# nagadomi/nunif

Hardware: NVIDIA H100
Metric: waifu2x_input_megapixels_per_sec (higher is better)
Workload: dtype f16

## Files before the change

### nunif_b200/csrc/gemm_wgmma.cuh

```cuda
#pragma once
#include "common.cuh"
#include "ptx.cuh"
#include <cuda.h>

namespace nb200 {

enum : int { ACT_NONE = 0, ACT_LRELU01 = 1, ACT_GELU = 2, ACT_RELU = 3 };
enum : int { OUT_NHWC = 0, OUT_PIXSHUF2 = 1, OUT_SPLIT = 2 };

struct GemmParams {
    int B, Ho, Wo, TH, TW, tiles_x, tiles_y;
    int N;
    int taps, cpt;
    int8_t tap_dx[16], tap_dy[16], tap_dyi[16];
    int n_tiles;
    const float* bias;
    int act;
    int out_mode, cout;
    int has_res, res_cy, res_cx;
    int res_before_act;
    int k2;
};

struct GemmMaps {
    CUtensorMap a, b;
    CUtensorMap o[4];
    union {
        CUtensorMap r[4];
        CUtensorMap a2;
    };
};

__device__ __forceinline__ void mbar_init(uint64_t* bar, uint32_t count) {
    asm volatile("mbarrier.init.shared::cta.b64 [%0], %1;" ::"r"(smem_u32(bar)), "r"(count));
}
__device__ __forceinline__ void mbar_expect_tx(uint64_t* bar, uint32_t bytes) {
    asm volatile("mbarrier.arrive.expect_tx.shared::cta.b64 _, [%0], %1;" ::"r"(smem_u32(bar)), "r"(bytes) : "memory");
}
__device__ __forceinline__ void mbar_arrive(uint64_t* bar) {
    asm volatile("mbarrier.arrive.shared::cta.b64 _, [%0];" ::"r"(smem_u32(bar)) : "memory");
}
static __device__ __noinline__ void mbar_timeout() {
    printf("nb200: mbarrier wait timed out (block %d,%d thread %d)\n", blockIdx.x, blockIdx.y, threadIdx.x);
    __trap();
}
__device__ __forceinline__ void mbar_wait(uint64_t* bar, uint32_t parity) {
    const uint32_t addr = smem_u32(bar);
    uint32_t done = 0;
#pragma unroll 1
    for (uint32_t it = 0; it < (1u << 18); ++it) {
        asm volatile(
            "{\n\t.reg .pred p;\n\t"
            "mbarrier.try_wait.parity.shared::cta.b64 p, [%1], %2, %3;\n\t"
            "selp.u32 %0, 1, 0, p;\n\t}"
            : "=r"(done) : "r"(addr), "r"(parity), "r"(20000u) : "memory");
        if (done) return;
    }
    mbar_timeout();
}
__device__ __forceinline__ void fence_barrier_init() {
    asm volatile("fence.mbarrier_init.release.cluster;" ::: "memory");
    asm volatile("fence.proxy.async.shared::cta;" ::: "memory");
}
__device__ __forceinline__ void tma_load_5d(const CUtensorMap* map, uint64_t* bar, void* dst, int c0, int c1, int c2, int c3, int c4) {
    asm volatile(
        "cp.async.bulk.tensor.5d.shared::cluster.global.tile.mbarrier::complete_tx::bytes [%0], [%1, {%3, %4, %5, %6, %7}], [%2];"
        ::"r"(smem_u32(dst)), "l"(map), "r"(smem_u32(bar)), "r"(c0), "r"(c1), "r"(c2), "r"(c3), "r"(c4) : "memory");
}
__device__ __forceinline__ void tma_load_2d(const CUtensorMap* map, uint64_t* bar, void* dst, int c0, int c1) {
    asm volatile(
        "cp.async.bulk.tensor.2d.shared::cluster.global.tile.mbarrier::complete_tx::bytes [%0], [%1, {%3, %4}], [%2];"
        ::"r"(smem_u32(dst)), "l"(map), "r"(smem_u32(bar)), "r"(c0), "r"(c1) : "memory");
}
__device__ __forceinline__ void tma_load_4d(const CUtensorMap* map, uint64_t* bar, void* dst, int c0, int c1, int c2, int c3) {
    asm volatile(
        "cp.async.bulk.tensor.4d.shared::cluster.global.tile.mbarrier::complete_tx::bytes [%0], [%1, {%3, %4, %5, %6}], [%2];"
        ::"r"(smem_u32(dst)), "l"(map), "r"(smem_u32(bar)), "r"(c0), "r"(c1), "r"(c2), "r"(c3) : "memory");
}
__device__ __forceinline__ void tma_store_4d(const CUtensorMap* map, const void* src, int c0, int c1, int c2, int c3) {
    asm volatile("cp.async.bulk.tensor.4d.global.shared::cta.tile.bulk_group [%0, {%2, %3, %4, %5}], [%1];"
                 ::"l"(map), "r"(smem_u32(src)), "r"(c0), "r"(c1), "r"(c2), "r"(c3) : "memory");
}
__device__ __forceinline__ void tma_store_2d(const CUtensorMap* map, const void* src, int c0, int c1) {
    asm volatile("cp.async.bulk.tensor.2d.global.shared::cta.tile.bulk_group [%0, {%2, %3}], [%1];"
                 ::"l"(map), "r"(smem_u32(src)), "r"(c0), "r"(c1) : "memory");
}
__device__ __forceinline__ void tma_store_commit() { asm volatile("cp.async.bulk.commit_group;" ::: "memory"); }
__device__ __forceinline__ void tma_store_wait_read() { asm volatile("cp.async.bulk.wait_group.read 0;" ::: "memory"); }
__device__ __forceinline__ void fence_async_smem() { asm volatile("fence.proxy.async.shared::cta;" ::: "memory"); }
__device__ __forceinline__ void consumer_bar_sync() { asm volatile("bar.sync 1, 256;" ::: "memory"); }
__device__ __forceinline__ void tma_prefetch_desc(const CUtensorMap* map) {
    asm volatile("prefetch.tensormap [%0];" ::"l"(map) : "memory");
}
__device__ __forceinline__ bool elect_one() {
    uint32_t pred;
    asm volatile(
        "{\n\t.reg .pred p;\n\t"
        "elect.sync _|p, 0xffffffff;\n\t"
        "selp.u32 %0, 1, 0, p;\n\t}"
        : "=r"(pred));
    return pred != 0;
}
__device__ __forceinline__ void wgmma_fence() { asm volatile("wgmma.fence.sync.aligned;" ::: "memory"); }
__device__ __forceinline__ void wgmma_commit() { asm volatile("wgmma.commit_group.sync.aligned;" ::: "memory"); }
template <int N>
__device__ __forceinline__ void wgmma_wait() { asm volatile("wgmma.wait_group.sync.aligned %0;" ::"n"(N) : "memory"); }
template <int K>
__device__ __forceinline__ void wgmma_fence_operands(float (&d)[K]) {
#pragma unroll
    for (int j = 0; j < K; ++j) asm volatile("" : "+f"(d[j])::"memory");
}
// ... 256 lines not shown
```

### nunif_b200/csrc/swin_attention_mma.cu

```cuda
#include "common.cuh"
#include "gemm_wgmma.cuh"
#include "swin_kernels.h"
#include "tmap.h"
#include <map>
#include <mutex>

namespace nb200 {

extern int g_tune[16];

namespace {
constexpr int WS = 6, WTOK = 36, WPAD = 48, HEADS = 6;
}

constexpr int NKT = 5;

template <int D>
struct AttnCtx {
    __half* sq;
    const int* sreg;
    const float4* bf;
    const __half* kbase[NKT];
    const __half* vbase[3];
    int hc, g, t4;
// ... 189 lines not shown
    }
    frag[i] = make_float4(v[0], v[1], v[2], v[3]);
}

int build_bias_frag(cudaStream_t st, const float* table, float* frag) {
    build_bias_frag_kernel<<<(HEADS * 3 * 6 * 32 + 255) / 256, 256, 0, st>>>(table, reinterpret_cast<float4*>(frag));
    NB_LAUNCHED();
    return 0;
}

template <int D>
static size_t attn_smem_bytes() {
    constexpr int C = D * HEADS, LD = C + 8;
    return (size_t)3 * WTOK * LD * 2 + (WTOK + WPAD) * 4 + 16;
}

static int set_attn_attrs(const void* func, size_t smem, int carveout) {
    static std::mutex mu;
    static std::map<std::pair<int, const void*>, int> done;
    int dev = 0;
    NB_CUDA(cudaGetDevice(&dev));
    std::lock_guard<std::mutex> lk(mu);
    int& have = done[{dev, func}];
    if (have != carveout) {
        NB_CUDA(cudaFuncSetAttribute(func, cudaFuncAttributeMaxDynamicSharedMemorySize, (int)smem));
        NB_CUDA(cudaFuncSetAttribute(func, cudaFuncAttributePreferredSharedMemoryCarveout, carveout));
        have = carveout;
    }
    return 0;
}

int window_attention(cudaStream_t st, const __half* qkv, const float* bias_frag_f, __half* out, int B, int H, int W, int C,
                     int shift, size_t plane) {
    const float4* bias_table = reinterpret_cast<const float4*>(bias_frag_f);
    NB_CHECK(H % WS == 0 && W % WS == 0, "feature map must be a multiple of the 6x6 window");
    NB_CHECK(C == 96 || C == 192, "window attention supports C=96 (d=16) and C=192 (d=32)");
    if (WS >= H) shift = 0;
    dim3 grid((H / WS) * (W / WS), B);
    ProfScope ps(st, PC_ATTN, (double)B * H * W * C * 4 * 2, (double)B * H * W * C * 3 * 2, (double)B * H * W * C * 2);
    if (C == 96) {
        const int want = g_tune[6] > 0 ? g_tune[6] : 72;
        if (set_attn_attrs((const void*)window_attention_mma_kernel<16>, attn_smem_bytes<16>(), want)) return 1;
        window_attention_mma_kernel<16><<<grid, 192, attn_smem_bytes<16>(), st>>>(qkv, bias_table, out, H, W, shift, plane);
    } else {
        const int want = g_tune[6] > 0 ? g_tune[6] : 86;
        if (set_attn_attrs((const void*)window_attention_mma_kernel<32>, attn_smem_bytes<32>(), want)) return 1;
        window_attention_mma_kernel<32><<<grid, 192, attn_smem_bytes<32>(), st>>>(qkv, bias_table, out, H, W, shift, plane);
    }
    NB_LAUNCHED();
    return 0;
}


constexpr int FA_ROWS = 128, FA_WIN = 3, FA_THREADS = GEMM_CONSUMER_THREADS + 32, FA_SLOT = 96 * 64, FA_STAGES = 4;
constexpr int FA_LD = 32 + 8;
constexpr int FA_CHUNK_BYTES = FA_WIN * 3 * WTOK * FA_LD * 2;

template <int C>
struct FaCfg {
    static constexpr int X_BYTES = FA_ROWS * C * 2;
    static constexpr int SMEM = X_BYTES + FA_STAGES * FA_SLOT + FA_CHUNK_BYTES + FA_WIN * (WTOK + WPAD) * 4 + 2 * FA_STAGES * 8 + 1024;
};

template <int C>
__global__ void __launch_bounds__(FA_THREADS, 2) swin_attn_fused_kernel(const __grid_constant__ CUtensorMap wmap,
                                                                        const __half* __restrict__ x, const float* __restrict__ bqkv,
                                                                        const float4* __restrict__ bias_frag, __half* __restrict__ out,
                                                                        int H, int W, int shift, int nwin) {
    using Cfg = FaCfg<C>;
    constexpr int D = C / HEADS, KB = C / 32, NCH = C / 32, HPC = 32 / D;
    extern __shared__ uint8_t smem_dyn[];
    uint8_t* smem = reinterpret_cast<uint8_t*>((reinterpret_cast<uintptr_t>(smem_dyn) + 1023) & ~(uintptr_t)1023);
    uint8_t* sx = smem;
    uint8_t* ring = smem + Cfg::X_BYTES;
    __half* sqkv = reinterpret_cast<__half*>(ring + FA_STAGES * FA_SLOT);
    int* stok = reinterpret_cast<int*>(reinterpret_cast<uint8_t*>(sqkv) + FA_CHUNK_BYTES);
    int* sreg = stok + FA_WIN * WTOK;
    uint64_t* full = reinterpret_cast<uint64_t*>(sreg + FA_WIN * WPAD);
    uint64_t* empty = full + FA_STAGES;
    const int tid = threadIdx.x, warp = tid >> 5;
    const int nww = W / WS, nwy = H / WS;
    if (tid < FA_WIN * WPAD) {
        const int w = tid / WPAD, t = tid % WPAD, gw = blockIdx.x * FA_WIN + w;
        int reg = -1;
        if (t < WTOK) {
            int tok = -1;
            if (gw < nwin) {
                const int b = gw / (nww * nwy), r = gw % (nww * nwy), wy = r / nww, wx = r % nww;
                const int ry = wy * WS + t / WS, rx = wx * WS + t % WS;
                const int y = (ry + shift) % H, xx = (rx + shift) % W;
                tok = (b * H + y) * W + xx;
                int hr = 0, wr = 0;
                if (shift > 0) {
                    hr = ry < H - WS ? 0 : (ry < H - shift ? 1 : 2);
                    wr = rx < W - WS ? 0 : (rx < W - shift ? 1 : 2);
                }
                reg = hr * 3 + wr;
            }
            stok[w * WTOK + t] = tok;
        }
        sreg[w * WPAD + t] = reg;
    }
    if (tid == GEMM_CONSUMER_THREADS) {
        tma_prefetch_desc(&wmap);
        for (int s = 0; s < FA_STAGES; ++s) {
            mbar_init(&full[s], 1);
            mbar_init(&empty[s], 2);
        }
        fence_barrier_init();
    }
    __syncthreads();
    if (tid == 0) NB_PDL_TRIGGER();

    if (warp == GEMM_CONSUMER_THREADS / 32) {
        if (elect_one()) {
            for (int i = 0; i < NCH * KB; ++i) {
                const int s = i % FA_STAGES, c = i / KB;
                mbar_wait(&empty[s], ((i / FA_STAGES) & 1) ^ 1);
                mbar_expect_tx(&full[s], FA_SLOT);
#pragma unroll
                for (int m = 0; m < 3; ++m)
                    tma_load_2d(&wmap, &full[s], ring + s * FA_SLOT + m * 32 * 64, (i % KB) * 32, m * C + 32 * c);
            }
        }
        return;
    }

    for (int i = tid; i < FA_ROWS * (C / 8); i += GEMM_CONSUMER_THREADS) {
        const int r = i / (C / 8), u = i % (C / 8);
        uint8_t* dst = sx + (u >> 2) * (FA_ROWS * 64) + stage_off<32>(r, u & 3);
        const int tok = r < FA_WIN * WTOK ? stok[r] : -1;
        if (tok >= 0) cp_async16(dst, x + (size_t)tok * C + u * 8);
        else *reinterpret_cast<uint4*>(dst) = make_uint4(0u, 0u, 0u, 0u);
    }
    cp_async_commit();
    cp_async_wait<0>();
    fence_async_smem();
    consumer_bar_sync();

    const int wg = tid >> 7, t = tid & 127;
    const int row0 = wg * 64 + (t >> 5) * 16 + ((t & 31) >> 2);
    const int cq = 2 * (t & 3);
    const uint32_t a_base = smem_u32(sx) + wg * 64 * 64;
    const int lane = tid & 31, g = lane >> 2, t4 = lane & 3;
    const float scale = ((D == 16) ? 0.25f : 0.17677669529663687f) * 1.4426950408889634f;
#pragma unroll 1
    for (int c = 0; c < NCH; ++c) {
        float acc[48];
#pragma unroll
        for (int j = 0; j < 48; ++j) acc[j] = 0.f;
#pragma unroll 1
        for (int kb = 0; kb < KB; ++kb) {
            const int it = c * KB + kb, s = it % FA_STAGES;
            mbar_wait(&full[s], (it / FA_STAGES) & 1);
            const uint32_t a = a_base + kb * (FA_ROWS * 64), bb = smem_u32(ring + s * FA_SLOT);
            wgmma_fence();
            wgmma_f16<96>(acc, make_kmajor_desc<64>(a), make_kmajor_desc<64>(bb), 1u);
            wgmma_f16<96>(acc, make_kmajor_desc<64>(a + 32), make_kmajor_desc<64>(bb + 32), 1u);
            wgmma_commit();
            wgmma_wait<1>();
            if (kb > 0 && t == 0) mbar_arrive(&empty[(it - 1) % FA_STAGES]);
        }
        wgmma_wait<0>();
        if (t == 0) mbar_arrive(&empty[(c * KB + KB - 1) % FA_STAGES]);
        wgmma_fence_operands(acc);
        consumer_bar_sync();
#pragma unroll
        for (int j = 0; j < 12; ++j) {
            const int m = j >> 2, col = 8 * (j & 3) + cq;
            const float2 bq = __ldg(reinterpret_cast<const float2*>(bqkv + m * C + 32 * c + col));
#pragma unroll
            for (int i = 0; i < 2; ++i) {
                const int r = row0 + 8 * i;
                if (r < FA_WIN * WTOK) {
                    const int w = r / WTOK, tk = r - w * WTOK;
                    *reinterpret_cast<__half2*>(sqkv + ((w * 3 + m) * WTOK + tk) * FA_LD + col) =
                        __floats2half2_rn(acc[4 * j + 2 * i] + bq.x, acc[4 * j + 2 * i + 1] + bq.y);
                }
            }
        }
        consumer_bar_sync();

#pragma unroll 1
        for (int item = warp; item < 3 * FA_WIN * HPC; item += GEMM_CONSUMER_THREADS / 32) {
            const int mt = item / (FA_WIN * HPC), pr = item - mt * (FA_WIN * HPC), w = pr / HPC, hh = pr - w * HPC;
            const int gw = blockIdx.x * FA_WIN + w;
            if (gw >= nwin) continue;
            const int r = gw % (nww * nwy), wy = r / nww, wx = r % nww, head = c * HPC + hh;
            __half* sq = sqkv + w * 3 * WTOK * FA_LD;
            __half* sk = sq + WTOK * FA_LD;
            __half* sv = sk + WTOK * FA_LD;
            AttnCtx<D> cx;
            cx.sq = sq; cx.sreg = sreg + w * WPAD; cx.bf = bias_frag + (size_t)head * (3 * 6 * 32) + lane;
            cx.hc = hh * D; cx.g = g; cx.t4 = t4; cx.scale = scale;
            cx.boundary = shift > 0 && (wy == nwy - 1 || wx == nww - 1);
#pragma unroll
            for (int nt = 0; nt < NKT; ++nt) cx.kbase[nt] = sk + min(nt * 8 + g, WTOK - 1) * FA_LD + cx.hc + 2 * t4;
            cx.vbase[0] = sv + (lane & 15) * FA_LD + cx.hc;
            cx.vbase[1] = sv + (16 + (lane & 15)) * FA_LD + cx.hc;
            cx.vbase[2] = sv + min(32 + (lane & 7), WTOK - 1) * FA_LD + cx.hc;
            if (mt < 2) attn_mtile<D, FA_LD, false>(cx, mt);
            else attn_mtile<D, FA_LD, true>(cx, 2);
            __syncwarp();
            const int nrow = mt < 2 ? 16 : WTOK - 32;
            for (int e = lane; e < nrow * (D / 8); e += 32) {
                const int tk = 16 * mt + e / (D / 8), u = e % (D / 8);
                *reinterpret_cast<uint4*>(out + (size_t)stok[w * WTOK + tk] * C + head * D + u * 8) =
                    *reinterpret_cast<const uint4*>(sq + tk * FA_LD + cx.hc + u * 8);
            }
        }
    }
}

int swin_attn_fused(cudaStream_t st, const __half* x, const __half* wqkv, const float* bqkv, const float* bias_frag_f, __half* att,
                    int B, int H, int W, int C, int shift) {
    NB_CHECK(x && wqkv && bqkv && bias_frag_f && att, "null pointer");
    NB_CHECK(H % WS == 0 && W % WS == 0, "feature map must be a multiple of the 6x6 window");
    NB_CHECK(C == 96 || C == 192, "fused window attention supports C=96 (d=16) and C=192 (d=32)");
    if (WS >= H) shift = 0;
    const long long nwin = (long long)B * (H / WS) * (W / WS);
    NB_CHECK(nwin > 0 && nwin < (1LL << 31), "window count out of range");
    CUtensorMap wmap;
    const cuuint64_t dims[2] = {(cuuint64_t)C, (cuuint64_t)(3 * C)};
    const cuuint64_t strides[1] = {(cuuint64_t)C * 2};
    const cuuint32_t box[2] = {32, 32};
    if (encode(&wmap, wqkv, 2, dims, strides, box, 64)) return 1;
    const double T = (double)B * H * W;
    ProfScope ps(st, PC_FUSED_ATTN, T * 3.0 * C * C * 2 + T * C * 36 * 4, T * C * 2, T * C * 2);
    const unsigned grid = (unsigned)((nwin + FA_WIN - 1) / FA_WIN);
    if (rec_on()) {
        char line[96];
        snprintf(line, sizeof(line), "swin_attn,%d,%d,%d,%d,%d", B, H, W, C, shift);
        rec_append(line);
    }
    const float4* bf = reinterpret_cast<const float4*>(bias_frag_f);
    if (C == 96) {
        if (ensure_dyn_smem((const void*)swin_attn_fused_kernel<96>, FaCfg<96>::SMEM)) return 1;
        swin_attn_fused_kernel<96><<<grid, FA_THREADS, FaCfg<96>::SMEM, st>>>(wmap, x, bqkv, bf, att, H, W, shift, (int)nwin);
    } else {
        if (ensure_dyn_smem((const void*)swin_attn_fused_kernel<192>, FaCfg<192>::SMEM)) return 1;
        swin_attn_fused_kernel<192><<<grid, FA_THREADS, FaCfg<192>::SMEM, st>>>(wmap, x, bqkv, bf, att, H, W, shift, (int)nwin);
    }
    NB_LAUNCHED();
    return 0;
}

}
```

### nunif_b200/csrc/swin_block.cu

```cuda
#include "gemm_wgmma.cuh"
#include "swin_kernels.h"
#include "tmap.h"

namespace nb200 {

constexpr int FM_ROWS = 128, FM_STAGES = 5, FM_THREADS = GEMM_CONSUMER_THREADS + 128;
constexpr int FM_PRODUCER_REGS = 40, FM_CONSUMER_REGS = 232;

template <int C>
struct FmCfg {
    static constexpr int KB = C / 32;
    static constexpr int TILE = FM_ROWS * C * 2;
    static constexpr int STAGE = 128 * C;
    static constexpr int SMEM = 2 * TILE + FM_STAGES * STAGE + (2 * FM_STAGES + KB + 1) * 8 + 1024;
};

struct FmMaps {
    CUtensorMap x, att, wp, w1, w2, y, wy;
};

template <int K>
__device__ __forceinline__ float (&half96(float (&acc)[K], int h))[48] { return *reinterpret_cast<float(*)[48]>(&acc[48 * h]); }

__device__ __forceinline__ void fm_wait(uint64_t* bar, uint32_t parity) {
    const uint32_t addr = smem_u32(bar);
    uint32_t done = 0;
#pragma unroll 1
    for (uint32_t it = 0; it < (1u << 18) && !done; ++it)
        asm volatile(
            "{\n\t.reg .pred p;\n\t"
            "mbarrier.try_wait.parity.shared::cta.b64 p, [%1], %2, %3;\n\t"
            "selp.u32 %0, 1, 0, p;\n\t}"
            : "=r"(done) : "r"(addr), "r"(parity), "r"(20000u) : "memory");
    if (!done) __trap();
}

__device__ __forceinline__ void wgmma_wait_n(int n) {
    if (n == 0) wgmma_wait<0>();
    else wgmma_wait<1>();
}

template <int C, bool PROJ, int CS>
__global__ void __launch_bounds__(FM_THREADS, 1) swin_mlp_fused_kernel(const __grid_constant__ FmMaps maps, const float* __restrict__ bp,
                                                                     const float* __restrict__ b1, const float* __restrict__ b2,
                                                                     const float* __restrict__ by) {
    using Cfg = FmCfg<C>;
    static_assert(CS % 16 == 0 && 2 * C * CS <= Cfg::STAGE && CS * 256 <= Cfg::TILE, "Wy must fit a ring stage, y the att tile");
    constexpr int KB = Cfg::KB, NP = (KB + 1) / 2, NH = 2 * C / 64, NHALF = C / 96;
    extern __shared__ uint8_t smem_dyn[];
    uint8_t* smem = reinterpret_cast<uint8_t*>((reinterpret_cast<uintptr_t>(smem_dyn) + 1023) & ~(uintptr_t)1023);
    uint8_t* sx = smem;
    uint8_t* satt = smem + Cfg::TILE;
    uint8_t* ring = smem + 2 * Cfg::TILE;
    uint64_t* full = reinterpret_cast<uint64_t*>(ring + FM_STAGES * Cfg::STAGE);
    uint64_t* empty = full + FM_STAGES;
    uint64_t* abar = empty + FM_STAGES;
    uint64_t* xbar = abar + KB;
    const int tid = threadIdx.x, warp = tid >> 5;
    const int row_base = blockIdx.x * FM_ROWS;
    if (tid == GEMM_CONSUMER_THREADS) {
        tma_prefetch_desc(&maps.x);
        tma_prefetch_desc(&maps.w1);
        tma_prefetch_desc(&maps.w2);
        if (CS) tma_prefetch_desc(&maps.wy);
        if (PROJ) {
            tma_prefetch_desc(&maps.att);
            tma_prefetch_desc(&maps.wp);
        }
        for (int s = 0; s < FM_STAGES; ++s) {
            mbar_init(&full[s], 1);
            mbar_init(&empty[s], 2);
        }
        for (int kb = 0; kb < KB; ++kb) mbar_init(&abar[kb], 1);
        mbar_init(xbar, 1);
        fence_barrier_init();
    }
    __syncthreads();

    if (warp >= GEMM_CONSUMER_THREADS / 32) {
        asm volatile("setmaxnreg.dec.sync.aligned.u32 %0;" ::"n"(FM_PRODUCER_REGS));
        if (warp == GEMM_CONSUMER_THREADS / 32 && elect_one()) {
            bool acts = false;
            auto load_acts = [&]() {
                asm volatile("griddepcontrol.wait;" ::: "memory");
                if (PROJ)
                    for (int kb = 0; kb < KB; ++kb) {
                        mbar_expect_tx(&abar[kb], FM_ROWS * 64);
                        tma_load_2d(&maps.att, &abar[kb], satt + kb * (FM_ROWS * 64), kb * 32, row_base);
                    }
                mbar_expect_tx(xbar, Cfg::TILE);
                for (int kb = 0; kb < KB; ++kb) tma_load_2d(&maps.x, xbar, sx + kb * (FM_ROWS * 64), kb * 32, row_base);
                acts = true;
            };
            int it = 0;
            auto push = [&](const CUtensorMap* m, int k0, int n0, int rows, int nbox) {
                if (it == FM_STAGES) load_acts();
                const int s = it % FM_STAGES;
                fm_wait(&empty[s], ((it / FM_STAGES) & 1) ^ 1);
                mbar_expect_tx(&full[s], nbox * rows * 64);
                for (int b = 0; b < nbox; ++b) tma_load_2d(m, &full[s], ring + s * Cfg::STAGE + b * rows * 64, k0 + 32 * b, n0);
                ++it;
            };
            if (PROJ)
                for (int j = 0; j < NP; ++j) push(&maps.wp, 64 * j, 0, C, min(2, KB - 2 * j));
            push(&maps.w1, 0, 0, 64, KB);
            for (int hc = 0; hc < NH; ++hc) {
                if (hc + 1 < NH) push(&maps.w1, 0, (hc + 1) * 64, 64, KB);
                push(&maps.w2, hc * 64, 0, C, 2);
            }
            if (CS) push(&maps.wy, 0, 0, CS, KB);
            if (!acts) load_acts();
        }
        return;
    }

    asm volatile("setmaxnreg.inc.sync.aligned.u32 %0;" ::"n"(FM_CONSUMER_REGS));
    const int wg = tid >> 7, t = tid & 127;
    const int row0 = wg * 64 + (t >> 5) * 16 + ((t & 31) >> 2);
    const int cq = 2 * (t & 3);
    const uint32_t x_base = smem_u32(sx) + wg * 64 * 64, att_base = smem_u32(satt) + wg * 64 * 64;
    int it = 0, pending = 0;
    auto take = [&]() -> uint32_t {
        const int s = it % FM_STAGES;
        fm_wait(&full[s], (it / FM_STAGES) & 1);
        return smem_u32(ring + s * Cfg::STAGE);
    };
    auto commit = [&]() {
        wgmma_commit();
        ++it;
        ++pending;
    };
    auto retire = [&](int n) {
        wgmma_wait_n(n);
#pragma unroll
        for (int k = 0; k < FM_STAGES; ++k)
            if (k < pending - n && t == 0) mbar_arrive(&empty[(it - pending + k) % FM_STAGES]);
        pending = min(pending, n);
    };

    if (PROJ) {
        float acc[C / 2];
#pragma unroll
        for (int j = 0; j < C / 2; ++j) acc[j] = 0.f;
        wgmma_fence_operands(acc);
#pragma unroll
        for (int j = 0; j < NP; ++j) {
            const uint32_t bb = take();
#pragma unroll
            for (int kb = 2 * j; kb < 2 * j + 2 && kb < KB; ++kb) fm_wait(&abar[kb], 0);
            wgmma_fence();
#pragma unroll
            for (int kb = 2 * j; kb < 2 * j + 2 && kb < KB; ++kb) {
                const uint32_t a = att_base + kb * (FM_ROWS * 64), b = bb + (kb - 2 * j) * (C * 64);
#pragma unroll
                for (int s = 0; s < 2; ++s)
#pragma unroll
                    for (int h = 0; h < NHALF; ++h)
                        wgmma_f16<96>(half96(acc, h), make_kmajor_desc<64>(a + 32 * s), make_kmajor_desc<64>(b + h * 96 * 64 + 32 * s), 1u);
            }
            commit();
            retire(1);
        }
        retire(0);
        wgmma_fence_operands(acc);
        fm_wait(xbar, 0);
#pragma unroll
        for (int j = 0; j < C / 8; ++j) {
            const int col = 8 * j + cq;
            const float2 bq = __ldg(reinterpret_cast<const float2*>(bp + col));
#pragma unroll
            for (int i = 0; i < 2; ++i) {
                __half2* p = reinterpret_cast<__half2*>(sx + sw64_off<FM_ROWS>(row0 + 8 * i, col));
                const float2 xv = __half22float2(*p);
                *p = __floats2half2_rn(xv.x + (acc[4 * j + 2 * i] + bq.x), xv.y + (acc[4 * j + 2 * i + 1] + bq.y));
            }
        }
        fence_async_smem();
        asm volatile("bar.sync %0, 128;" ::"r"(2 + wg) : "memory");
    } else {
        fm_wait(xbar, 0);
    }

    float oacc[C / 2];
#pragma unroll
    for (int j = 0; j < C / 2; ++j) oacc[j] = 0.f;
    wgmma_fence_operands(oacc);
    float hacc[2][32];
    uint32_t af[4][4];
    auto fc1 = [&](float (&h)[32]) {
#pragma unroll
        for (int j = 0; j < 32; ++j) h[j] = 0.f;
        wgmma_fence_operands(h);
        const uint32_t bb = take();
        wgmma_fence();
#pragma unroll
        for (int kb = 0; kb < KB; ++kb) {
            const uint32_t a = x_base + kb * (FM_ROWS * 64), b = bb + kb * (64 * 64);
            wgmma_f16<64>(h, make_kmajor_desc<64>(a), make_kmajor_desc<64>(b), 1u);
            wgmma_f16<64>(h, make_kmajor_desc<64>(a + 32), make_kmajor_desc<64>(b + 32), 1u);
        }
        commit();
    };
    fc1(hacc[0]);
#pragma unroll
    for (int hc = 0; hc < NH; ++hc) {
        const int buf = hc & 1;
        if (hc + 1 < NH) fc1(hacc[buf ^ 1]);
        retire(hc + 1 < NH ? 1 : 0);
        wgmma_fence_operands(hacc[buf]);
#pragma unroll
        for (int kk = 0; kk < 4; ++kk)
#pragma unroll
            for (int q = 0; q < 4; ++q) {
                const int j = 2 * kk + (q >> 1), i = q & 1;
                const float2 bq = __ldg(reinterpret_cast<const float2*>(b1 + 64 * hc + 8 * j + cq));
                af[kk][q] = pack_half2(gelu_erf(hacc[buf][4 * j + 2 * i] + bq.x), gelu_erf(hacc[buf][4 * j + 2 * i + 1] + bq.y));
            }
        const uint32_t bb = take();
        wgmma_fence();
#pragma unroll
        for (int kb = 0; kb < 2; ++kb)
#pragma unroll
            for (int s = 0; s < 2; ++s)
#pragma unroll
                for (int h = 0; h < NHALF; ++h)
                    wgmma_f16_rs96(half96(oacc, h), af[2 * kb + s], make_kmajor_desc<64>(bb + kb * (C * 64) + h * 96 * 64 + 32 * s), 1u);
        commit();
    }
    retire(0);
    wgmma_fence_operands(oacc);
#pragma unroll
    for (int j = 0; j < C / 8; ++j) {
        const int col = 8 * j + cq;
// ... 136 lines not shown
```

### profiles/ab_swin_attn.py

```python
#!/usr/bin/env python
import argparse
import ctypes
import json
import os
import statistics
import subprocess
import sys
import tempfile

ROOT = os.path.dirname(os.path.dirname(os.path.abspath(__file__)))
sys.path.insert(0, ROOT)

SHAPES = [(240, 96), (120, 192), (60, 192), (240, 192)]
BATCH = 16
REPS = 7
WINDOW_MS = 60.0
FA_THREADS = 288
KERNEL = "_ZN5nb20022swin_attn_fused_kernelILi{C}EEEv14CUtensorMap_stPK6__halfPKfPK6float4PS2_iiii"


def load(path):
    from nunif_b200 import _lib
    lib = ctypes.CDLL(os.path.abspath(path))
    for name in ("nb200_last_error", "nb200_check_device", "nb200_swin_attn_fused_f16"):
        res, args = _lib.SIGNATURES[name]
        getattr(lib, name).restype, getattr(lib, name).argtypes = res, args
    return lib


def check(lib, rc):
    if rc != 0:
        raise RuntimeError(lib.nb200_last_error().decode("utf-8", "replace"))


def call(lib, t, shift):
    import torch
    x, wqkv, bqkv, table, att = t
    B, H, W, C = x.shape
    p = lambda v: ctypes.c_void_p(v.data_ptr())
    check(lib, lib.nb200_swin_attn_fused_f16(p(x), p(wqkv), p(bqkv), p(table), p(att), B, H, W, C, shift,
                                             ctypes.c_void_p(torch.cuda.current_stream().cuda_stream)))


def inputs(H, C, shift, dev):
    import torch
    g = torch.Generator(device="cpu").manual_seed(H * 1000 + C + shift)
    x = torch.randn(BATCH, H, H, C, generator=g).half().to(dev)
    wqkv = (torch.randn(3 * C, C, generator=g) / C ** 0.5).half().to(dev)
    bqkv = (0.1 * torch.randn(3 * C, generator=g)).to(dev)
    table = (0.5 * torch.randn(121, 6, generator=g)).to(dev)
    return x, wqkv, bqkv, table


def window_ms(lib, t, shift, n):
    import torch
    e0, e1 = torch.cuda.Event(enable_timing=True), torch.cuda.Event(enable_timing=True)
    e0.record()
    for _ in range(n):
        call(lib, t, shift)
    e1.record()
    e1.synchronize()
    return e0.elapsed_time(e1) / n


def launch_smem(libs, dev):
    import torch
    from torch.profiler import ProfilerActivity, profile
    out = {}
    with tempfile.TemporaryDirectory() as d:
        for tag, lib in libs.items():
            for C in (96, 192):
                x, wqkv, bqkv, table = inputs(12, C, 0, dev)
                t = (x, wqkv, bqkv, table, torch.empty_like(x))
                with profile(activities=[ProfilerActivity.CUDA]) as prof:
                    call(lib, t, 0)
                    torch.cuda.synchronize()
                path = os.path.join(d, f"{tag}{C}.json")
                prof.export_chrome_trace(path)
                ev = [e for e in json.load(open(path))["traceEvents"]
                      if e.get("cat") == "kernel" and "swin_attn_fused_kernel" in e.get("name", "")]
                a = ev[0]["args"]
                out[(tag, C)] = {"smem": int(a["shared memory"]), "regs_trace": int(a["registers per thread"])}
    return out


def occupancy(so_path, C, smem):
    name = KERNEL.format(C=C)
    cuobjdump = os.path.join(os.environ.get("CUDA_HOME", "/usr/local/cuda"), "bin", "cuobjdump")
    with tempfile.TemporaryDirectory() as d:
        subprocess.run([cuobjdump, "-xelf", "all", os.path.abspath(so_path)], cwd=d, check=True, capture_output=True)
        image = next(b for b in (open(os.path.join(d, f), "rb").read() for f in sorted(os.listdir(d))) if name.encode() in b)
    cu = ctypes.CDLL("libcuda.so.1")

    def ck(rc):
        if rc != 0:
            raise RuntimeError(f"CUDA driver error {rc}")
    mod, fn = ctypes.c_void_p(), ctypes.c_void_p()
    ck(cu.cuModuleLoadData(ctypes.byref(mod), ctypes.c_char_p(image)))
    try:
        ck(cu.cuModuleGetFunction(ctypes.byref(fn), mod, name.encode()))
        ck(cu.cuFuncSetAttribute(fn, 8, ctypes.c_int(smem)))
        regs, n = ctypes.c_int(), ctypes.c_int()
        ck(cu.cuFuncGetAttribute(ctypes.byref(regs), 4, fn))
        ck(cu.cuOccupancyMaxActiveBlocksPerMultiprocessor(ctypes.byref(n), fn, FA_THREADS, ctypes.c_size_t(smem)))
    finally:
        cu.cuModuleUnload(mod)
    return regs.value, n.value


def device_info(index):
    q = subprocess.run(["nvidia-smi", "-i", str(index), "--query-gpu=name,power.limit,clocks.max.sm", "--format=csv,noheader"],
                       capture_output=True, text=True)
    return q.stdout.strip()


def main():
    ap = argparse.ArgumentParser(description=__doc__, formatter_class=argparse.RawDescriptionHelpFormatter)
    ap.add_argument("--base", required=True, help="the build to compare against (libnunif_b200.so)")
    ap.add_argument("--new", default=os.path.join(ROOT, "nunif_b200", "libnunif_b200.so"), help="default: this tree's build")
    ap.add_argument("--out", default=None, help="also write the JSON result here")
    args = ap.parse_args()
    import torch
    from bench import ClockSampler
    dev = torch.device("cuda:0")
    torch.cuda.init()
    torch.zeros(1, device=dev)
    paths = {"base": args.base, "new": args.new}
    libs = {k: load(v) for k, v in paths.items()}
    for lib in libs.values():
        check(lib, lib.nb200_check_device(0))
    info = {"device": torch.cuda.get_device_name(dev), "nvidia_smi": device_info(0), "paths": paths}
    print(f"# {info['device']} | name, power limit, max SM clock: {info['nvidia_smi']}")

    kern = []
    try:
        for (tag, C), s in sorted(launch_smem(libs, dev).items()):
            regs, ctas = occupancy(paths[tag], C, s["smem"])
            kern.append({"build": tag, "C": C, "regs": regs, "dyn_smem": s["smem"], "ctas_per_sm": ctas})
            print(f"# {tag:4s} swin_attn_fused_kernel<{C}>: {regs} registers, {s['smem']} B shared memory/CTA, {ctas} CTA(s)/SM")
    except Exception as e:
        kern.append({"error": f"{type(e).__name__}: {e}"})
        print(f"# occupancy query failed: {type(e).__name__}: {e}")

    rows = []
    with torch.inference_mode(), ClockSampler(0) as clocks:
        for H, C in SHAPES:
            for shift in (0, 3):
                x, wqkv, bqkv, table = inputs(H, C, shift, dev)
                t = {k: (x, wqkv, bqkv, table, torch.full_like(x, 7.0)) for k in libs}
                for k, lib in libs.items():
                    for _ in range(3):
                        call(lib, t[k], shift)
                torch.cuda.synchronize()
                equal = torch.equal(t["base"][4], t["new"][4])
                diff = float((t["base"][4].float() - t["new"][4].float()).abs().max())
                est = max(window_ms(libs["base"], t["base"], shift, 2), window_ms(libs["new"], t["new"], shift, 2))
                n = max(3, int(WINDOW_MS / max(est, 1e-3)))
                ms = {k: [] for k in libs}
                for r in range(REPS):
                    for k in (("base", "new") if r % 2 == 0 else ("new", "base")):
                        ms[k].append(window_ms(libs[k], t[k], shift, n))
                row = {"B": BATCH, "H": H, "W": H, "C": C, "shift": shift, "calls_per_window": n, "equal": equal, "max_abs_diff": diff}
                for k in libs:
                    row[k] = {"median_ms": statistics.median(ms[k]), "min_ms": min(ms[k]), "max_ms": max(ms[k])}
                row["new_over_base"] = row["new"]["median_ms"] / row["base"]["median_ms"]
                rows.append(row)
                b, nw = row["base"], row["new"]
                print(f"{BATCH}x{H}x{H}x{C} shift {shift}: base {b['median_ms']:.4f} ms [{b['min_ms']:.4f}, {b['max_ms']:.4f}]  "
                      f"new {nw['median_ms']:.4f} ms [{nw['min_ms']:.4f}, {nw['max_ms']:.4f}]  new/base {row['new_over_base']:.3f}  "
                      f"outputs {'identical' if equal else f'DIFFER (max |d| {diff:g})'}", flush=True)
                del t, x
    result = {"info": info, "clocks": clocks.summary(), "kernels": kern, "shapes": rows,
              "all_equal": all(r["equal"] for r in rows)}
    print(json.dumps(result))
    if args.out:
        os.makedirs(os.path.dirname(os.path.abspath(args.out)), exist_ok=True)
        with open(args.out, "w") as fh:
            json.dump(result, fh, indent=1)
    return 0 if result["all_equal"] else 1


if __name__ == "__main__":
    sys.exit(main())
```

Baseline: 71.18.

## Make fused swin attention persistent with warp-specialized QKV GEMM and attention pipeline

The fused window-attention kernel becomes persistent, with the grid capped at the SM count. Work is split into a TMA producer warp, wgmma consumer warpgroups that compute the QKV projection, and 11 dedicated attention warps. These roles hand off through double-buffered activation tiles and QKV chunks guarded by mbarriers, so the next tile's gather and GEMM overlap the current tile's attention instead of running serially under block-wide barriers. Ring stages now hold three K-blocks each, and token indices are recomputed rather than kept in shared memory. The cost is one CTA per SM with larger shared memory and a more complex synchronization scheme. The mbarrier wait helper is also unified, dropping the printf timeout path.

After: 74.04 (median of 6 runs). 4.0% higher.

```diff
diff --git a/nunif_b200/csrc/gemm_wgmma.cuh b/nunif_b200/csrc/gemm_wgmma.cuh
--- a/nunif_b200/csrc/gemm_wgmma.cuh
+++ b/nunif_b200/csrc/gemm_wgmma.cuh
@@ -40,23 +40,17 @@
 __device__ __forceinline__ void mbar_arrive(uint64_t* bar) {
     asm volatile("mbarrier.arrive.shared::cta.b64 _, [%0];" ::"r"(smem_u32(bar)) : "memory");
 }
-static __device__ __noinline__ void mbar_timeout() {
-    printf("nb200: mbarrier wait timed out (block %d,%d thread %d)\n", blockIdx.x, blockIdx.y, threadIdx.x);
-    __trap();
-}
 __device__ __forceinline__ void mbar_wait(uint64_t* bar, uint32_t parity) {
     const uint32_t addr = smem_u32(bar);
     uint32_t done = 0;
 #pragma unroll 1
-    for (uint32_t it = 0; it < (1u << 18); ++it) {
+    for (uint32_t it = 0; it < (1u << 18) && !done; ++it)
         asm volatile(
             "{\n\t.reg .pred p;\n\t"
             "mbarrier.try_wait.parity.shared::cta.b64 p, [%1], %2, %3;\n\t"
             "selp.u32 %0, 1, 0, p;\n\t}"
             : "=r"(done) : "r"(addr), "r"(parity), "r"(20000u) : "memory");
-        if (done) return;
-    }
-    mbar_timeout();
+    if (!done) __trap();
 }
 __device__ __forceinline__ void fence_barrier_init() {
     asm volatile("fence.mbarrier_init.release.cluster;" ::: "memory");
diff --git a/nunif_b200/csrc/swin_attention_mma.cu b/nunif_b200/csrc/swin_attention_mma.cu
--- a/nunif_b200/csrc/swin_attention_mma.cu
+++ b/nunif_b200/csrc/swin_attention_mma.cu
@@ -265,162 +265,241 @@
 }
 
 
-constexpr int FA_ROWS = 128, FA_WIN = 3, FA_THREADS = GEMM_CONSUMER_THREADS + 32, FA_SLOT = 96 * 64, FA_STAGES = 4;
+constexpr int FA_ROWS = 128, FA_WIN = 3, FA_SLOT = 96 * 64, FA_KPS = 3, FA_STAGES = 4;
+constexpr int FA_MMA_THREADS = GEMM_CONSUMER_THREADS, FA_PRODUCER_WARP = FA_MMA_THREADS / 32, FA_ATTN_WARPS = 11;
+constexpr int FA_THREADS = FA_MMA_THREADS + 32 + 32 * FA_ATTN_WARPS;
 constexpr int FA_LD = 32 + 8;
 constexpr int FA_CHUNK_BYTES = FA_WIN * 3 * WTOK * FA_LD * 2;
+constexpr int FA_STAGE = FA_KPS * FA_SLOT;
 
 template <int C>
 struct FaCfg {
     static constexpr int X_BYTES = FA_ROWS * C * 2;
-    static constexpr int SMEM = X_BYTES + FA_STAGES * FA_SLOT + FA_CHUNK_BYTES + FA_WIN * (WTOK + WPAD) * 4 + 2 * FA_STAGES * 8 + 1024;
+    static constexpr int SMEM = 2 * X_BYTES + FA_STAGES * FA_STAGE + 2 * FA_CHUNK_BYTES + 4 * WPAD * 4 + (2 * FA_STAGES + 8) * 8 + 1024;
 };
 
+__device__ __forceinline__ int fa_token(int b, int wy, int wx, int t, int H, int W, int shift) {
+    int y = wy * WS + t / WS + shift, xx = wx * WS + t % WS + shift;
+    if (y >= H) y -= H;
+    if (xx >= W) xx -= W;
+    return (b * H + y) * W + xx;
+}
+
 template <int C>
-__global__ void __launch_bounds__(FA_THREADS, 2) swin_attn_fused_kernel(const __grid_constant__ CUtensorMap wmap,
+__global__ void __launch_bounds__(FA_THREADS, 1) swin_attn_fused_kernel(const __grid_constant__ CUtensorMap wmap,
                                                                         const __half* __restrict__ x, const float* __restrict__ bqkv,
                                                                         const float4* __restrict__ bias_frag, __half* __restrict__ out,
                                                                         int H, int W, int shift, int nwin) {
     using Cfg = FaCfg<C>;
     constexpr int D = C / HEADS, KB = C / 32, NCH = C / 32, HPC = 32 / D;
+    constexpr int IPC = 3 * FA_WIN * HPC, IPT = NCH * IPC;
+    constexpr int SPC = KB / FA_KPS;
+    constexpr int VPR = C / 8;
+    static_assert(KB % FA_KPS == 0, "a ring stage holds FA_KPS K-blocks of one chunk");
+    static_assert(FA_WIN == 3, "the gather selects among 3 windows");
     extern __shared__ uint8_t smem_dyn[];
     uint8_t* smem = reinterpret_cast<uint8_t*>((reinterpret_cast<uintptr_t>(smem_dyn) + 1023) & ~(uintptr_t)1023);
     uint8_t* sx = smem;
-    uint8_t* ring = smem + Cfg::X_BYTES;
-    __half* sqkv = reinterpret_cast<__half*>(ring + FA_STAGES * FA_SLOT);
-    int* stok = reinterpret_cast<int*>(reinterpret_cast<uint8_t*>(sqkv) + FA_CHUNK_BYTES);
-    int* sreg = stok + FA_WIN * WTOK;
-    uint64_t* full = reinterpret_cast<uint64_t*>(sreg + FA_WIN * WPAD);
+    uint8_t* ring = smem + 2 * Cfg::X_BYTES;
+    __half* schunk = reinterpret_cast<__half*>(ring + FA_STAGES * FA_STAGE);
+    int* sreg = reinterpret_cast<int*>(reinterpret_cast<uint8_t*>(schunk) + 2 * FA_CHUNK_BYTES);
+    uint64_t* full = reinterpret_cast<uint64_t*>(sreg + 4 * WPAD);
     uint64_t* empty = full + FA_STAGES;
-    const int tid = threadIdx.x, warp = tid >> 5;
+    uint64_t* afull = empty + FA_STAGES;
+    uint64_t* aempty = afull + 2;
+    uint64_t* cfull = aempty + 2;
+    uint64_t* cempty = cfull + 2;
+    const int tid = threadIdx.x, warp = tid >> 5, lane = tid & 31;
     const int nww = W / WS, nwy = H / WS;
-    if (tid < FA_WIN * WPAD) {
-        const int w = tid / WPAD, t = tid % WPAD, gw = blockIdx.x * FA_WIN + w;
+    const int ntiles = (nwin + FA_WIN - 1) / FA_WIN;
+    const int ntl = (ntiles - (int)blockIdx.x + (int)gridDim.x - 1) / (int)gridDim.x;
+
+    if (tid < 4 * WPAD) {
+        const int p = tid / WPAD, t = tid % WPAD;
         int reg = -1;
         if (t < WTOK) {
-            int tok = -1;
-            if (gw < nwin) {
-                const int b = gw / (nww * nwy), r = gw % (nww * nwy), wy = r / nww, wx = r % nww;
-                const int ry = wy * WS + t / WS, rx = wx * WS + t % WS;
-                const int y = (ry + shift) % H, xx = (rx + shift) % W;
-                tok = (b * H + y) * W + xx;
-                int hr = 0, wr = 0;
-                if (shift > 0) {
-                    hr = ry < H - WS ? 0 : (ry < H - shift ? 1 : 2);
-                    wr = rx < W - WS ? 0 : (rx < W - shift ? 1 : 2);
-                }
-                reg = hr * 3 + wr;
-            }
-            stok[w * WTOK + t] = tok;
-        }
-        sreg[w * WPAD + t] = reg;
-    }
-    if (tid == GEMM_CONSUMER_THREADS) {
+            const int hr = (p & 2) ? (t / WS < WS - shift ? 1 : 2) : 0;
+            const int wr = (p & 1) ? (t % WS < WS - shift ? 1 : 2) : 0;
+            reg = hr * 3 + wr;
+        }
+        sreg[tid] = reg;
+    }
+    for (int i = tid; i < 2 * (FA_ROWS - FA_WIN * WTOK) * VPR; i += FA_THREADS) {
+        const int bsel = i / ((FA_ROWS - FA_WIN * WTOK) * VPR), j = i % ((FA_ROWS - FA_WIN * WTOK) * VPR);
+        const int r = FA_WIN * WTOK + j / VPR, u = j % VPR;
+        *reinterpret_cast<uint4*>(sx + bsel * Cfg::X_BYTES + (u >> 2) * (FA_ROWS * 64) + stage_off<32>(r, u & 3)) =
+            make_uint4(0u, 0u, 0u, 0u);
+    }
+    if (tid == FA_MMA_THREADS) {
         tma_prefetch_desc(&wmap);
         for (int s = 0; s < FA_STAGES; ++s) {
             mbar_init(&full[s], 1);
             mbar_init(&empty[s], 2);
         }
+        for (int b = 0; b < 2; ++b) {
+            mbar_init(&afull[b], 32 * FA_ATTN_WARPS);
+            mbar_init(&aempty[b], 2);
+            mbar_init(&cfull[b], FA_MMA_THREADS / 32);
+            mbar_init(&cempty[b], IPC);
+        }
         fence_barrier_init();
     }
+    fence_async_smem();
     __syncthreads();
     if (tid == 0) NB_PDL_TRIGGER();
 
-    if (warp == GEMM_CONSUMER_THREADS / 32) {
+    if (warp == FA_PRODUCER_WARP) {
         if (elect_one()) {
-            for (int i = 0; i < NCH * KB; ++i) {
-                const int s = i % FA_STAGES, c = i / KB;
-                mbar_wait(&empty[s], ((i / FA_STAGES) & 1) ^ 1);
-                mbar_expect_tx(&full[s], FA_SLOT);
-#pragma unroll
-                for (int m = 0; m < 3; ++m)
-                    tma_load_2d(&wmap, &full[s], ring + s * FA_SLOT + m * 32 * 64, (i % KB) * 32, m * C + 32 * c);
+            int q = 0;
+#pragma unroll 1
+            for (int k = 0; k < ntl; ++k) {
+#pragma unroll 1
+                for (int i = 0; i < NCH * SPC; ++i, ++q) {
+                    const int s = q % FA_STAGES, c = i / SPC, kb0 = (i % SPC) * FA_KPS;
+                    mbar_wait(&empty[s], ((q / FA_STAGES) & 1) ^ 1);
+                    mbar_expect_tx(&full[s], FA_STAGE);
+#pragma unroll
+                    for (int kk = 0; kk < FA_KPS; ++kk)
+#pragma unroll
+                        for (int m = 0; m < 3; ++m)
+                            tma_load_2d(&wmap, &full[s], ring + s * FA_STAGE + kk * FA_SLOT + m * 32 * 64, (kb0 + kk) * 32, m * C + 32 * c);
+                }
             }
         }
         return;
     }
 
-    for (int i = tid; i < FA_ROWS * (C / 8); i += GEMM_CONSUMER_THREADS) {
-        const int r = i / (C / 8), u = i % (C / 8);
-        uint8_t* dst = sx + (u >> 2) * (FA_ROWS * 64) + stage_off<32>(r, u & 3);
-        const int tok = r < FA_WIN * WTOK ? stok[r] : -1;
-        if (tok >= 0) cp_async16(dst, x + (size_t)tok * C + u * 8);
-        else *reinterpret_cast<uint4*>(dst) = make_uint4(0u, 0u, 0u, 0u);
-    }
-    cp_async_commit();
-    cp_async_wait<0>();
-    fence_async_smem();
-    consumer_bar_sync();
+    const float scale = ((D == 16) ? 0.25f : 0.17677669529663687f) * 1.4426950408889634f;
+    const int g = lane >> 2, t4 = lane & 3;
+    if (warp > FA_PRODUCER_WARP) {
+        const int aw = warp - FA_PRODUCER_WARP - 1;
+        auto gather = [&](int tile, uint8_t* sa) {
+            int wb[FA_WIN], wwy[FA_WIN], wwx[FA_WIN];
+#pragma unroll
+            for (int w = 0; w < FA_WIN; ++w) {
+                const int gw = tile * FA_WIN + w, b = gw / (nww * nwy), rw = gw - b * (nww * nwy);
+                wb[w] = gw < nwin ? b : -1;
+                wwy[w] = rw / nww;
+                wwx[w] = rw - wwy[w] * nww;
+            }
+            for (int i = aw * 32 + lane; i < FA_WIN * WTOK * VPR; i += 32 * FA_ATTN_WARPS) {
+                const int r = i / VPR, u = i % VPR, w = r / WTOK;
+                const int b = w == 0 ? wb[0] : (w == 1 ? wb[1] : wb[2]);
+                const int wy = w == 0 ? wwy[0] : (w == 1 ? wwy[1] : wwy[2]), wx = w == 0 ? wwx[0] : (w == 1 ? wwx[1] : wwx[2]);
+                uint8_t* dst = sa + (u >> 2) * (FA_ROWS * 64) + stage_off<32>(r, u & 3);
+                if (b >= 0) cp_async16(dst, x + (size_t)fa_token(b, wy, wx, r - w * WTOK, H, W, shift) * C + u * 8);
+                else *reinterpret_cast<uint4*>(dst) = make_uint4(0u, 0u, 0u, 0u);
+            }
+            cp_async_commit();
+        };
+        auto gathered = [&](int kt) {
+            cp_async_wait<0>();
+            fence_async_smem();
+            mbar_arrive(&afull[kt & 1]);
+        };
+        gather(blockIdx.x, sx);
+        gathered(0);
+        int kcur = -1, nth = 0;
+#pragma unroll 1
+        for (int n = aw; n < ntl * IPT; n += FA_ATTN_WARPS) {
+            const int gc = n / IPC, item = n - gc * IPC, c = gc % NCH;
+            const int kt = n / IPT, tile = blockIdx.x + kt * gridDim.x;
+            mbar_wait(&cfull[gc & 1], (gc >> 1) & 1);
+            if (kt != kcur) {
+                kcur = kt;
+                nth = 0;
+            }
+            if (kt + 1 < ntl && nth == 0) {
+                mbar_wait(&aempty[(kt + 1) & 1], (((kt + 1) >> 1) & 1) ^ 1);
+                gather(tile + gridDim.x, sx + ((kt + 1) & 1) * Cfg::X_BYTES);
+            }
+            if (kt + 1 < ntl && nth == 1) gathered(kt + 1);
+            ++nth;
+            const int mt = item / (FA_WIN * HPC), pr = item - mt * (FA_WIN * HPC), w = pr / HPC, hh = pr - w * HPC;
+            const int gw = tile * FA_WIN + w;
+            if (gw < nwin) {
+                const int b = gw / (nww * nwy), r = gw % (nww * nwy), wy = r / nww, wx = r % nww, head = c * HPC + hh;
+                const bool lrow = wy == nwy - 1, lcol = wx == nww - 1;
+                __half* sq = schunk + (gc & 1) * (FA_CHUNK_BYTES / 2) + w * 3 * WTOK * FA_LD;
+                __half* sk = sq + WTOK * FA_LD;
+                __half* sv = sk + WTOK * FA_LD;
+                AttnCtx<D> cx;
+                cx.sq = sq; cx.sreg = sreg + (2 * lrow + lcol) * WPAD; cx.bf = bias_frag + (size_t)head * (3 * 6 * 32) + lane;
+                cx.hc = hh * D; cx.g = g; cx.t4 = t4; cx.scale = scale;
+                cx.boundary = shift > 0 && (lrow || lcol);
+#pragma unroll
+                for (int nt = 0; nt < NKT; ++nt) cx.kbase[nt] = sk + min(nt * 8 + g, WTOK - 1) * FA_LD + cx.hc + 2 * t4;
+                cx.vbase[0] = sv + (lane & 15) * FA_LD + cx.hc;
+                cx.vbase[1] = sv + (16 + (lane & 15)) * FA_LD + cx.hc;
+                cx.vbase[2] = sv + min(32 + (lane & 7), WTOK - 1) * FA_LD + cx.hc;
+                if (mt < 2) attn_mtile<D, FA_LD, false>(cx, mt);
+                else attn_mtile<D, FA_LD, true>(cx, 2);
+                __syncwarp();
+                const int nrow = mt < 2 ? 16 : WTOK - 32;
+                for (int e = lane; e < nrow * (D / 8); e += 32) {
+                    const int tk = 16 * mt + e / (D / 8), u = e % (D / 8);
+                    *reinterpret_cast<uint4*>(out + (size_t)fa_token(b, wy, wx, tk, H, W, shift) * C + head * D + u * 8) =
+                        *reinterpret_cast<const uint4*>(sq + tk * FA_LD + cx.hc + u * 8);
+                }
+            }
+            __syncwarp();
+            if (lane == 0) mbar_arrive(&cempty[gc & 1]);
+        }
+        return;
+    }
 
     const int wg = tid >> 7, t = tid & 127;
     const int row0 = wg * 64 + (t >> 5) * 16 + ((t & 31) >> 2);
     const int cq = 2 * (t & 3);
-    const uint32_t a_base = smem_u32(sx) + wg * 64 * 64;
-    const int lane = tid & 31, g = lane >> 2, t4 = lane & 3;
-    const float scale = ((D == 16) ? 0.25f : 0.17677669529663687f) * 1.4426950408889634f;
-#pragma unroll 1
-    for (int c = 0; c < NCH; ++c) {
-        float acc[48];
-#pragma unroll
-        for (int j = 0; j < 48; ++j) acc[j] = 0.f;
-#pragma unroll 1
-        for (int kb = 0; kb < KB; ++kb) {
-            const int it = c * KB + kb, s = it % FA_STAGES;
-            mbar_wait(&full[s], (it / FA_STAGES) & 1);
-            const uint32_t a = a_base + kb * (FA_ROWS * 64), bb = smem_u32(ring + s * FA_SLOT);
-            wgmma_fence();
-            wgmma_f16<96>(acc, make_kmajor_desc<64>(a), make_kmajor_desc<64>(bb), 1u);
-            wgmma_f16<96>(acc, make_kmajor_desc<64>(a + 32), make_kmajor_desc<64>(bb + 32), 1u);
-            wgmma_commit();
-            wgmma_wait<1>();
-            if (kb > 0 && t == 0) mbar_arrive(&empty[(it - 1) % FA_STAGES]);
-        }
-        wgmma_wait<0>();
-        if (t == 0) mbar_arrive(&empty[(c * KB + KB - 1) % FA_STAGES]);
-        wgmma_fence_operands(acc);
-        consumer_bar_sync();
-#pragma unroll
-        for (int j = 0; j < 12; ++j) {
-            const int m = j >> 2, col = 8 * (j & 3) + cq;
-            const float2 bq = __ldg(reinterpret_cast<const float2*>(bqkv + m * C + 32 * c + col));
-#pragma unroll
-            for (int i = 0; i < 2; ++i) {
-                const int r = row0 + 8 * i;
-                if (r < FA_WIN * WTOK) {
-                    const int w = r / WTOK, tk = r - w * WTOK;
-                    *reinterpret_cast<__half2*>(sqkv + ((w * 3 + m) * WTOK + tk) * FA_LD + col) =
-                        __floats2half2_rn(acc[4 * j + 2 * i] + bq.x, acc[4 * j + 2 * i + 1] + bq.y);
+    int q = 0, gc = 0;
+#pragma unroll 1
+    for (int k = 0; k < ntl; ++k) {
+        mbar_wait(&afull[k & 1], (k >> 1) & 1);
+        const uint32_t a_base = smem_u32(sx + (k & 1) * Cfg::X_BYTES) + wg * 64 * 64;
+#pragma unroll 1
+        for (int c = 0; c < NCH; ++c, ++gc) {
+            float acc[48];
+#pragma unroll
+            for (int j = 0; j < 48; ++j) acc[j] = 0.f;
+#pragma unroll 1
+            for (int j = 0; j < SPC; ++j, ++q) {
+                const int s = q % FA_STAGES;
+                mbar_wait(&full[s], (q / FA_STAGES) & 1);
+                wgmma_fence();
+#pragma unroll
+                for (int kk = 0; kk < FA_KPS; ++kk) {
+                    const uint32_t a = a_base + (j * FA_KPS + kk) * (FA_ROWS * 64), bb = smem_u32(ring + s * FA_STAGE + kk * FA_SLOT);
+                    wgmma_f16<96>(acc, make_kmajor_desc<64>(a), make_kmajor_desc<64>(bb), 1u);
+                    wgmma_f16<96>(acc, make_kmajor_desc<64>(a + 32), make_kmajor_desc<64>(bb + 32), 1u);
                 }
-            }
-        }
-        consumer_bar_sync();
-
-#pragma unroll 1
-        for (int item = warp; item < 3 * FA_WIN * HPC; item += GEMM_CONSUMER_THREADS / 32) {
-            const int mt = item / (FA_WIN * HPC), pr = item - mt * (FA_WIN * HPC), w = pr / HPC, hh = pr - w * HPC;
-            const int gw = blockIdx.x * FA_WIN + w;
-            if (gw >= nwin) continue;
-            const int r = gw % (nww * nwy), wy = r / nww, wx = r % nww, head = c * HPC + hh;
-            __half* sq = sqkv + w * 3 * WTOK * FA_LD;
-            __half* sk = sq + WTOK * FA_LD;
-            __half* sv = sk + WTOK * FA_LD;
-            AttnCtx<D> cx;
-            cx.sq = sq; cx.sreg = sreg + w * WPAD; cx.bf = bias_frag + (size_t)head * (3 * 6 * 32) + lane;
-            cx.hc = hh * D; cx.g = g; cx.t4 = t4; cx.scale = scale;
-            cx.boundary = shift > 0 && (wy == nwy - 1 || wx == nww - 1);
-#pragma unroll
-            for (int nt = 0; nt < NKT; ++nt) cx.kbase[nt] = sk + min(nt * 8 + g, WTOK - 1) * FA_LD + cx.hc + 2 * t4;
-            cx.vbase[0] = sv + (lane & 15) * FA_LD + cx.hc;
-            cx.vbase[1] = sv + (16 + (lane & 15)) * FA_LD + cx.hc;
-            cx.vbase[2] = sv + min(32 + (lane & 7), WTOK - 1) * FA_LD + cx.hc;
-            if (mt < 2) attn_mtile<D, FA_LD, false>(cx, mt);
-            else attn_mtile<D, FA_LD, true>(cx, 2);
+                wgmma_commit();
+                wgmma_wait<1>();
+                if (j > 0 && t == 0) mbar_arrive(&empty[(q - 1) % FA_STAGES]);
+            }
+            wgmma_wait<0>();
+            if (t == 0) {
+                mbar_arrive(&empty[(q - 1) % FA_STAGES]);
+                if (c == NCH - 1) mbar_arrive(&aempty[k & 1]);
+            }
+            wgmma_fence_operands(acc);
+            mbar_wait(&cempty[gc & 1], ((gc >> 1) & 1) ^ 1);
+            __half* sqkv = schunk + (gc & 1) * (FA_CHUNK_BYTES / 2);
+#pragma unroll
+            for (int j = 0; j < 12; ++j) {
+                const int m = j >> 2, col = 8 * (j & 3) + cq;
+                const float2 bq = __ldg(reinterpret_cast<const float2*>(bqkv + m * C + 32 * c + col));
+#pragma unroll
+                for (int i = 0; i < 2; ++i) {
+                    const int r = row0 + 8 * i;
+                    if (r < FA_WIN * WTOK) {
+                        const int w = r / WTOK, tk = r - w * WTOK;
+                        *reinterpret_cast<__half2*>(sqkv + ((w * 3 + m) * WTOK + tk) * FA_LD + col) =
+                            __floats2half2_rn(acc[4 * j + 2 * i] + bq.x, acc[4 * j + 2 * i + 1] + bq.y);
+                    }
+                }
+            }
             __syncwarp();
-            const int nrow = mt < 2 ? 16 : WTOK - 32;
-            for (int e = lane; e < nrow * (D / 8); e += 32) {
-                const int tk = 16 * mt + e / (D / 8), u = e % (D / 8);
-                *reinterpret_cast<uint4*>(out + (size_t)stok[w * WTOK + tk] * C + head * D + u * 8) =
-                    *reinterpret_cast<const uint4*>(sq + tk * FA_LD + cx.hc + u * 8);
-            }
+            if (lane == 0) mbar_arrive(&cfull[gc & 1]);
         }
     }
 }
@@ -440,7 +519,8 @@
     if (encode(&wmap, wqkv, 2, dims, strides, box, 64)) return 1;
     const double T = (double)B * H * W;
     ProfScope ps(st, PC_FUSED_ATTN, T * 3.0 * C * C * 2 + T * C * 36 * 4, T * C * 2, T * C * 2);
-    const unsigned grid = (unsigned)((nwin + FA_WIN - 1) / FA_WIN);
+    const long long ntiles = (nwin + FA_WIN - 1) / FA_WIN;
+    const unsigned grid = (unsigned)std::min<long long>(ntiles, device_sm_count());
     if (rec_on()) {
         char line[96];
         snprintf(line, sizeof(line), "swin_attn,%d,%d,%d,%d,%d", B, H, W, C, shift);
diff --git a/nunif_b200/csrc/swin_block.cu b/nunif_b200/csrc/swin_block.cu
--- a/nunif_b200/csrc/swin_block.cu
+++ b/nunif_b200/csrc/swin_block.cu
@@ -21,19 +21,6 @@
 
 template <int K>
 __device__ __forceinline__ float (&half96(float (&acc)[K], int h))[48] { return *reinterpret_cast<float(*)[48]>(&acc[48 * h]); }
-
-__device__ __forceinline__ void fm_wait(uint64_t* bar, uint32_t parity) {
-    const uint32_t addr = smem_u32(bar);
-    uint32_t done = 0;
-#pragma unroll 1
-    for (uint32_t it = 0; it < (1u << 18) && !done; ++it)
-        asm volatile(
-            "{\n\t.reg .pred p;\n\t"
-            "mbarrier.try_wait.parity.shared::cta.b64 p, [%1], %2, %3;\n\t"
-            "selp.u32 %0, 1, 0, p;\n\t}"
-            : "=r"(done) : "r"(addr), "r"(parity), "r"(20000u) : "memory");
-    if (!done) __trap();
-}
 
 __device__ __forceinline__ void wgmma_wait_n(int n) {
     if (n == 0) wgmma_wait<0>();
@@ -96,7 +83,7 @@
             auto push = [&](const CUtensorMap* m, int k0, int n0, int rows, int nbox) {
                 if (it == FM_STAGES) load_acts();
                 const int s = it % FM_STAGES;
-                fm_wait(&empty[s], ((it / FM_STAGES) & 1) ^ 1);
+                mbar_wait(&empty[s], ((it / FM_STAGES) & 1) ^ 1);
                 mbar_expect_tx(&full[s], nbox * rows * 64);
                 for (int b = 0; b < nbox; ++b) tma_load_2d(m, &full[s], ring + s * Cfg::STAGE + b * rows * 64, k0 + 32 * b, n0);
                 ++it;
@@ -122,7 +109,7 @@
     int it = 0, pending = 0;
     auto take = [&]() -> uint32_t {
         const int s = it % FM_STAGES;
-        fm_wait(&full[s], (it / FM_STAGES) & 1);
+        mbar_wait(&full[s], (it / FM_STAGES) & 1);
         return smem_u32(ring + s * Cfg::STAGE);
     };
     auto commit = [&]() {
@@ -147,7 +134,7 @@
         for (int j = 0; j < NP; ++j) {
             const uint32_t bb = take();
 #pragma unroll
-            for (int kb = 2 * j; kb < 2 * j + 2 && kb < KB; ++kb) fm_wait(&abar[kb], 0);
+            for (int kb = 2 * j; kb < 2 * j + 2 && kb < KB; ++kb) mbar_wait(&abar[kb], 0);
             wgmma_fence();
 #pragma unroll
             for (int kb = 2 * j; kb < 2 * j + 2 && kb < KB; ++kb) {
@@ -163,7 +150,7 @@
         }
         retire(0);
         wgmma_fence_operands(acc);
-        fm_wait(xbar, 0);
+        mbar_wait(xbar, 0);
 #pragma unroll
         for (int j = 0; j < C / 8; ++j) {
             const int col = 8 * j + cq;
@@ -178,7 +165,7 @@
         fence_async_smem();
         asm volatile("bar.sync %0, 128;" ::"r"(2 + wg) : "memory");
     } else {
-        fm_wait(xbar, 0);
+        mbar_wait(xbar, 0);
     }
 
     float oacc[C / 2];
diff --git a/profiles/ab_swin_attn.py b/profiles/ab_swin_attn.py
--- a/profiles/ab_swin_attn.py
+++ b/profiles/ab_swin_attn.py
@@ -15,7 +15,6 @@
 BATCH = 16
 REPS = 7
 WINDOW_MS = 60.0
-FA_THREADS = 288
 KERNEL = "_ZN5nb20022swin_attn_fused_kernelILi{C}EEEv14CUtensorMap_stPK6__halfPKfPK6float4PS2_iiii"
 
 
@@ -80,11 +79,12 @@
                 ev = [e for e in json.load(open(path))["traceEvents"]
                       if e.get("cat") == "kernel" and "swin_attn_fused_kernel" in e.get("name", "")]
                 a = ev[0]["args"]
-                out[(tag, C)] = {"smem": int(a["shared memory"]), "regs_trace": int(a["registers per thread"])}
+                out[(tag, C)] = {"smem": int(a["shared memory"]), "regs_trace": int(a["registers per thread"]),
+                                 "threads": a["block"][0] * a["block"][1] * a["block"][2]}
     return out
 
 
-def occupancy(so_path, C, smem):
+def occupancy(so_path, C, smem, threads):
     name = KERNEL.format(C=C)
     cuobjdump = os.path.join(os.environ.get("CUDA_HOME", "/usr/local/cuda"), "bin", "cuobjdump")
     with tempfile.TemporaryDirectory() as d:
@@ -102,7 +102,7 @@
         ck(cu.cuFuncSetAttribute(fn, 8, ctypes.c_int(smem)))
         regs, n = ctypes.c_int(), ctypes.c_int()
         ck(cu.cuFuncGetAttribute(ctypes.byref(regs), 4, fn))
-        ck(cu.cuOccupancyMaxActiveBlocksPerMultiprocessor(ctypes.byref(n), fn, FA_THREADS, ctypes.c_size_t(smem)))
+        ck(cu.cuOccupancyMaxActiveBlocksPerMultiprocessor(ctypes.byref(n), fn, threads, ctypes.c_size_t(smem)))
     finally:
         cu.cuModuleUnload(mod)
     return regs.value, n.value
@@ -135,9 +135,10 @@
     kern = []
     try:
         for (tag, C), s in sorted(launch_smem(libs, dev).items()):
-            regs, ctas = occupancy(paths[tag], C, s["smem"])
-            kern.append({"build": tag, "C": C, "regs": regs, "dyn_smem": s["smem"], "ctas_per_sm": ctas})
-            print(f"# {tag:4s} swin_attn_fused_kernel<{C}>: {regs} registers, {s['smem']} B shared memory/CTA, {ctas} CTA(s)/SM")
+            regs, ctas = occupancy(paths[tag], C, s["smem"], s["threads"])
+            kern.append({"build": tag, "C": C, "regs": regs, "dyn_smem": s["smem"], "threads": s["threads"], "ctas_per_sm": ctas})
+            print(f"# {tag:4s} swin_attn_fused_kernel<{C}>: {s['threads']} threads, {regs} registers, {s['smem']} B shared memory/CTA, "
+                  f"{ctas} CTA(s)/SM")
     except Exception as e:
         kern.append({"error": f"{type(e).__name__}: {e}"})
         print(f"# occupancy query failed: {type(e).__name__}: {e}")
```
